# marcinp7/music-style-transfer

Hardware: AMD Instinct MI355X
Metric: style-transfer opt iters/sec (higher is better)
Workload: dtype f32; 1 GPU; one 30 s clip per GPU (BASELINE.json configs[1]): piano-roll C=4,R=16,T=4 (+percussion), full widths (980325 params), fwd+loss+bwd every step, Adam+StepLR every iter_size steps; clips_per_gpu=1, iter_size=2, hip_graph=True, graphs=one joint graph, accumulation=2 concurrent streams, launches_per_pass=71, parallelism=single GPU

## Files before the change

include/mst_amd.h:

```cpp
#ifndef MST_AMD_H
#define MST_AMD_H
#include <stdint.h>

#ifdef __cplusplus
extern "C" {
#endif

typedef enum {
    MST_OK = 0,
    MST_ERR_ARG = -1,
    MST_ERR_UNSUPPORTED = -2,
    MST_ERR_LAUNCH = -3,
    MST_ERR_ALLOC = -4,
} mst_status;

typedef struct {
    int32_t C, R, T;
    int32_t beat, bar, nrf;
    int32_t style, melody, rhythm;
    int32_t instr;
    int32_t n_instruments;
    int32_t has_unpitched;
    int32_t clips;
} mst_dims;
// ... 122 lines not shown
                          const int32_t* rows , int32_t n_clips,
                          const mst_row_fields* fields ,
                          int64_t clip_stride, float* ws, mst_stream stream);

#define MST_EVAL_ACC_WORDS (2 + MST_N_LOSSES + 3 * MST_METRIC_WORDS)
int32_t mst_eval_accumulate(const float* losses   ,
                            const double* metrics ,
                            int32_t n_clips, int32_t channels,
                            const int32_t* live   ,
                            double* acc , mst_stream stream);

int32_t mst_plan_step_count(const mst_plan* p, int32_t stage_mask, int32_t backward);
int32_t mst_plan_step_info(const mst_plan* p, int32_t stage_mask, int32_t backward, int32_t* info );
int32_t mst_plan_step_carried(const mst_plan* p, int32_t stage_mask, int32_t backward, int32_t* carried);
int32_t mst_plan_step_riders(const mst_plan* p, int32_t stage_mask, int32_t backward, int32_t* out);
int32_t mst_plan_zero_rides(const mst_plan* p);
int32_t mst_plan_step_carrier(const mst_plan* p, int32_t stage_mask, int32_t backward, int32_t* out);
int32_t mst_plan_set_lstm_small(mst_plan* p, int32_t on);
int32_t mst_plan_step_gemms(const mst_plan* p, int32_t stage_mask, int32_t backward, int32_t step, int32_t* out, int32_t cap);
int32_t mst_plan_time_steps(const mst_plan* p, int32_t stage_mask, int32_t backward, const float* params,
                            float* gparams, float* ws, const float* pitched, const float* unpitched,
                            mst_stream stream, int32_t reps, float* ms, int32_t* kind, double* flops, double* bytes);

typedef struct mst_audio_plan mst_audio_plan;
mst_audio_plan* mst_audio_plan_create(int32_t n_fft , int32_t hop, int64_t n_samples, int32_t* status);
void mst_audio_plan_destroy(mst_audio_plan* p);
int32_t mst_audio_plan_info(const mst_audio_plan* p, int64_t out[6]);
int32_t mst_audio_stft(const mst_audio_plan* p, const float* audio, float* spec, float* mag, mst_stream stream);
int32_t mst_audio_gram(const mst_audio_plan* p, const float* feat, float* gram, float* ws, mst_stream stream);
int32_t mst_audio_style_iteration(const mst_audio_plan* p, float* x, const float* gram_style, float* grad, float* exp_avg,
                                  float* exp_avg_sq, float* state, float* ws, float* loss, double lr, mst_stream stream);

int32_t mst_debug_slab_columns_disjoint(int64_t off_x, int32_t width_x, int64_t off_y, int32_t width_y, int32_t ld);

const char* mst_version(void);

#ifdef __cplusplus
}
#endif
#endif
```

music-style-transfer_amd/csrc/gemm.hip:

```cpp
#include "combine_body.h"
#include "lstm_small_body.h"

__device__ __forceinline__ float act_fwd(int act, float z, int col) {
    if (act == ACT_LEAKY) return z > 0.f ? z : z * LEAKY;
    if (act == ACT_SIGOUT) { float s = 1.f / (1.f + expf(-z)); return col == 0 ? 6.f * s : s; }
    if (act == ACT_BPM) { float s = 1.f / (1.f + expf(-z)); return s * 150.f + 50.f; }
    return z;
}

__device__ __forceinline__ float act_bwd(int act, float y, int col) {
    if (act == ACT_LEAKY) return y > 0.f ? 1.f : LEAKY;
    if (act == ACT_SIGOUT) return col == 0 ? y * (1.f - y * (1.f / 6.f)) : y * (1.f - y);
    if (act == ACT_BPM) { float s = (y - 50.f) * (1.f / 150.f); return 150.f * s * (1.f - s); }
    return 1.f;
}

typedef const MST_GLOBAL_AS float* gcptr;
#define GEMM_PAD 1

template <int KIND>
__device__ __forceinline__ int off_of(const Operand& o, int i, int j, bool& ok) {
    if constexpr (KIND == OPK_DENSE) {
        return i * (int)o.si + j * (int)o.sj;
    } else if constexpr (KIND == OPK_ACTGRAD) {
        return o.transposed ? j * o.ld + i : i * o.ld + j;
    } else if constexpr (KIND == OPK_IM2COL) {
        const int p = i >> 3, oc = i & 7;
        const int f = j / (CONV_K * NPF), rem = j - f * (CONV_K * NPF);
        const int e = (NDEG * oc - CONV_PAD) * NPF + rem;
        ok = ok & (e >= 0) & (e < NPN * NPF);
        return p * (NF * NPN * NPF) + f * (NPN * NPF) + e;
    } else if constexpr (KIND == OPK_PERMW) {
        if (o.pb == CONV_K && o.pc == NPF) {
            constexpr int BC = CONV_K * NPF;
            const int a = i / BC, rem = i - a * BC;
            const int bb = rem / NPF, c = rem - bb * NPF;
            return j * o.ld + a * BC + c * CONV_K + bb;
        }
        if (o.pb == NUN && o.pc == NUF) {
            constexpr int BC = NUN * NUF;
            const int a = i / BC, rem = i - a * BC;
            const int bb = rem / NUF, c = rem - bb * NUF;
            return j * o.ld + a * BC + c * NUN + bb;
        }
        const int bc = o.pb * o.pc;
        const int a = i / bc, rem = i - a * bc;
        const int bb = rem / o.pc, c = rem - bb * o.pc;
        return j * o.ld + a * bc + c * o.pb + bb;
    } else {
        return (j >> 3) * (o.oc * NOCT) + i * NOCT + (j & 7);
    }
}

template <int OK>
__device__ __forceinline__ void store_out(const GemmDesc& d, float* cbase, const float* bias, int m, int n, int split, float acc) {
    const OutSpec& o = d.out;
    if constexpr (OK == OUT_STORE) {
        float v = acc;
        if (bias) v += o.bias_div > 0 ? bias[(unsigned)((m / o.bias_div) * o.bias_ld + n)] : bias[n];
        cbase[(unsigned)(m * o.ldc + n)] = act_fwd(o.act, v, n);
    } else if constexpr (OK == OUT_ACCUM) {
        float* c = cbase + (unsigned)(m * o.ldc + n);
        *c = o.first ? acc : *c + acc;
    } else if constexpr (OK == OUT_CONV) {
        cbase[(unsigned)((m >> 3) * o.ldc + n * NOCT + (m & 7))] = act_fwd(ACT_LEAKY, acc + bias[n], 0);
    } else if constexpr (OK == OUT_SLAB) {
        const unsigned idx = n < o.wcols ? (unsigned)(m * o.wcols + n) : (unsigned)(d.M * o.wcols + m);
        cbase[(int64_t)split * o.slab_stride + idx] = acc;
    } else {
        unsigned idx;
        if (n < o.wcols) {
            int a, bb, c, bc;
            if (o.pb == CONV_K && o.pc == NPF) { bc = CONV_K * NPF; a = n / (CONV_K * NPF); const int rem = n - a * (CONV_K * NPF); bb = rem / NPF; c = rem - bb * NPF; }
            else if (o.pb == NUN && o.pc == NUF) { bc = NUN * NUF; a = n / (NUN * NUF); const int rem = n - a * (NUN * NUF); bb = rem / NUF; c = rem - bb * NUF; }
            else { bc = o.pb * o.pc; a = n / bc; const int rem = n - a * bc; bb = rem / o.pc; c = rem - bb * o.pc; }
            idx = (unsigned)(m * o.wcols + a * bc + c * o.pb + bb);
        } else {
            idx = (unsigned)(d.M * o.wcols + m);
        }
        cbase[(int64_t)split * o.slab_stride + idx] = acc;
    }
}

template <int AK, int BKIND, int OK, int AKF, int BKF, int KD>
__device__ __forceinline__ void gemm_body(const GemmDesc& d, const Bases& b, const int tile, const int split,
                                          float (*As)[GEMM_BM + GEMM_PAD], float (*Bs)[GEMM_BN + GEMM_PAD]) {
    const int tid = threadIdx.x;
    const int M = d.M, N = d.N;
    const int tiles_n = (N + GEMM_BN - 1) / GEMM_BN;
    const gcptr baseA = (gcptr)(b.p[d.A.space] + d.A.off);
    const gcptr baseA2 = (AK == OPK_ACTGRAD || AK == OPK_CONVGRAD) ? (gcptr)(b.p[d.A.space2] + d.A.off2) : baseA;
    const gcptr baseB = (gcptr)(b.p[d.B.space] + d.B.off);
    const int tm = tile / tiles_n, tn = tile - tm * tiles_n;
    int kchunk = (d.K + d.ksplit - 1) / d.ksplit;
    kchunk = (kchunk + KD - 1) / KD * KD;
    const int k0 = split * kchunk;
    const int k1 = min(d.K, k0 + kchunk);
    const int wv = tid >> 6, lane = tid & 63;
    const int a_act = (AK == OPK_ACTGRAD) ? d.A.act : ACT_LEAKY;
    const int a_tr = d.A.transposed;
    const int b_ones = (BKIND == OPK_DENSE || BKIND == OPK_IM2COL) ? d.B.ones_at : -1;
    typedef float acc_f32x16 __attribute__((ext_vector_type(16)));
    acc_f32x16 acc;
#pragma unroll
    for (int r = 0; r < 16; ++r) acc[r] = 0.f;

    constexpr int NT = GEMM_THREADS, NW = NT / 64;
    constexpr int NL = GEMM_BM * KD / NT;
    constexpr int KW = KD / NW;
    float va[NL], ya[NL], vb[NL];

#define A_ROW(i) (AKF ? (tid / KD) + (NT / KD) * (i) : (tid & 31))
#define A_KL(i) (AKF ? (tid % KD) : (tid >> 5) + (NT / 32) * (i))
#define B_ROW(i) (BKF ? (tid / KD) + (NT / KD) * (i) : (tid & 31))
#define B_KL(i) (BKF ? (tid % KD) : (tid >> 5) + (NT / 32) * (i))
#define GEMM_ISSUE(KT)                                                                                     \
    {                                                                                                      \
        _Pragma("unroll") for (int i = 0; i < NL; ++i) {                                                   \
            const int m = tm * GEMM_BM + A_ROW(i), ka = (KT) + A_KL(i);                                    \
            bool oka = (m < M) & (ka < k1);                                                                \
            int ia = off_of<AK>(d.A, m, ka, oka);                                                          \
            ia = oka ? ia : 0;                                                                             \
            const float x = baseA[(unsigned)ia];                                                           \
            if constexpr (AK == OPK_ACTGRAD || AK == OPK_CONVGRAD) {                                       \
                const float y = baseA2[(unsigned)ia];                                                      \
                const int col = (AK == OPK_ACTGRAD) ? (a_tr ? m : ka) : 0;                                 \
                ya[i] = act_bwd(a_act, y, col);                                                            \
            } else ya[i] = 1.f;                                                                            \
            va[i] = oka ? x : 0.f;                                                                         \
            const int n = tn * GEMM_BN + B_ROW(i), kb = (KT) + B_KL(i);                                    \
            bool okb = (n < N) & (kb < k1);                                                                \
            const bool one = okb & (n == b_ones);                                                          \
            int ib = off_of<BKIND>(d.B, kb, n, okb);                                                       \
            ib = (okb & !one) ? ib : 0;                                                                    \
            const float w = baseB[(unsigned)ib];                                                           \
            vb[i] = one ? 1.f : (okb ? w : 0.f);                                                           \
        }                                                                                                  \
    }

    if (k0 < k1) GEMM_ISSUE(k0)
    for (int kt = k0; kt < k1; kt += KD) {
#pragma unroll
        for (int i = 0; i < NL; ++i) {
            As[A_KL(i)][A_ROW(i)] = (AK == OPK_ACTGRAD || AK == OPK_CONVGRAD) ? va[i] * ya[i] : va[i];
            Bs[B_KL(i)][B_ROW(i)] = vb[i];
        }
        __syncthreads();
        if (kt + KD < k1) GEMM_ISSUE(kt + KD)
#pragma unroll
        for (int kk = 0; kk < KW; kk += 2) {
            const int k = wv * KW + kk + (lane >> 5);
            acc = __builtin_amdgcn_mfma_f32_32x32x2f32(As[k][lane & 31], Bs[k][lane & 31], acc, 0, 0, 0);
        }
        __syncthreads();
    }
#undef GEMM_ISSUE
#undef A_ROW
#undef A_KL
#undef B_ROW
#undef B_KL
    float* red = &As[0][0];
#pragma unroll
    for (int r = 0; r < 16; ++r)
        red[wv * (GEMM_BM * GEMM_BN) + ((r & 3) + 8 * (r >> 2) + 4 * (lane >> 5)) * GEMM_BN + (lane & 31)] = acc[r];
    __syncthreads();
    float* cbase = b.p[d.out.space] + d.out.off;
    const float* bias = d.out.bias_space >= 0 ? b.p[d.out.bias_space] + d.out.bias_off : nullptr;
#pragma unroll
    for (int q = 0; q < GEMM_BM * GEMM_BN / NT; ++q) {
        const int o = tid + q * NT;
// ... 496 lines not shown
        return;
    }
    lb -= seg_blocks;
    if (lb < gat_blocks) {
        const int m = lb / r.gat_blocks;
        gather_rows<GATHER_RIDER_ROWS>(r.gathers[clip * r.gat_members + m], lb - m * r.gat_blocks, r.gat_blocks, b);
        return;
    }
    lb -= gat_blocks;
    if (lb < r.zero_chunks) {
        const ZeroChunk c = r.zero[lb];
        float* p = b.p[SP_GRAD] + (int64_t)clip * r.zero_stride + c.off;
        for (int i = threadIdx.x; i < c.len; i += GEMM_THREADS) p[i] = 0.f;
    }
}

__global__ __launch_bounds__(GEMM_THREADS) void gemm_kernel(const GemmDesc* __restrict__ descs, const int* __restrict__ owner, int count, int blocks_per_clip, int rider_blocks, Bases b, GemmRiders r) {
    constexpr int TILE_F = GEMM_BK * (GEMM_BM + GEMM_PAD), RED_F = (GEMM_THREADS / 64) * GEMM_BM * GEMM_BN;
    __shared__ __attribute__((aligned(16))) float smem[(2 * TILE_F > RED_F) ? 2 * TILE_F : RED_F];
    float (*As)[GEMM_BM + GEMM_PAD] = reinterpret_cast<float (*)[GEMM_BM + GEMM_PAD]>(smem);
    float (*Bs)[GEMM_BN + GEMM_PAD] = reinterpret_cast<float (*)[GEMM_BN + GEMM_PAD]>(smem + TILE_F);
    const int clip = blockIdx.x / blocks_per_clip;
    int lb = blockIdx.x - clip * blocks_per_clip;
    if (lb < rider_blocks) {
        gemm_rider_block(r, clip, lb, b, smem);
        return;
    }
    lb -= rider_blocks;
    const int lo = owner[lb];
    const GemmDesc d = descs[clip * count + lo];
    const int local = lb - d.blk_begin;
    const int ntile = ((d.M + GEMM_BM - 1) / GEMM_BM) * ((d.N + GEMM_BN - 1) / GEMM_BN);
    const int tile = local % ntile, split = local / ntile;
#define GEMM_CASE(V, A_, B_, O_, AF_, BF_)                                                          \
    case (V) * 3 + 0: gemm_body<A_, B_, O_, AF_, BF_, 32>(d, b, tile, split, As, Bs); break;           \
    case (V) * 3 + 1: gemm_body<A_, B_, O_, AF_, BF_, 64>(d, b, tile, split, As, Bs); break;           \
    case (V) * 3 + 2: gemm_body<A_, B_, O_, AF_, BF_, 128>(d, b, tile, split, As, Bs); break;
    switch (d.variant * 3 + d.kdsel) {
        GEMM_CASE(GV_LIN_FWD, OPK_DENSE, OPK_DENSE, OUT_STORE, 1, 1)
        GEMM_CASE(GV_LIN_FWD_PERM, OPK_DENSE, OPK_PERMW, OUT_STORE, 1, 1)
        GEMM_CASE(GV_LIN_DW, OPK_ACTGRAD, OPK_DENSE, OUT_SLAB, 0, 0)
        GEMM_CASE(GV_LIN_DW_PERM, OPK_ACTGRAD, OPK_DENSE, OUT_PERMW_SLAB, 0, 0)
        GEMM_CASE(GV_LIN_DA, OPK_ACTGRAD, OPK_DENSE, OUT_ACCUM, 1, 0)
        GEMM_CASE(GV_CONV_FWD, OPK_IM2COL, OPK_PERMW, OUT_CONV, 1, 1)
        GEMM_CASE(GV_CONV_DW, OPK_CONVGRAD, OPK_IM2COL, OUT_PERMW_SLAB, 1, 0)
        GEMM_CASE(GV_HH_DW, OPK_DENSE, OPK_DENSE, OUT_SLAB, 0, 0)
        GEMM_CASE(GV_LIN_DA_RAW, OPK_DENSE, OPK_DENSE, OUT_ACCUM, 1, 0)
    default: break;
    }
#undef GEMM_CASE
}

int gemm_variant(const GemmDesc& g) {
    const int a = g.A.kind, bk = g.B.kind, o = g.out.kind;
    if (a == OPK_DENSE && bk == OPK_DENSE && o == OUT_STORE) return GV_LIN_FWD;
    if (a == OPK_DENSE && bk == OPK_PERMW && o == OUT_STORE) return GV_LIN_FWD_PERM;
    if (a == OPK_ACTGRAD && bk == OPK_DENSE && o == OUT_SLAB) return GV_LIN_DW;
    if (a == OPK_ACTGRAD && bk == OPK_DENSE && o == OUT_PERMW_SLAB) return GV_LIN_DW_PERM;
    if (a == OPK_ACTGRAD && bk == OPK_DENSE && o == OUT_ACCUM) return GV_LIN_DA;
    if (a == OPK_IM2COL && bk == OPK_PERMW && o == OUT_CONV) return GV_CONV_FWD;
    if (a == OPK_CONVGRAD && bk == OPK_IM2COL && o == OUT_PERMW_SLAB) return GV_CONV_DW;
    if (a == OPK_DENSE && bk == OPK_DENSE && o == OUT_SLAB) return GV_HH_DW;
    if (a == OPK_DENSE && bk == OPK_DENSE && o == OUT_ACCUM) return GV_LIN_DA_RAW;
    return -1;
}

int gemm_rider_blocks(const GemmRiders& r) { return r.lstm_members * r.lstm_blocks + r.comb[0].sites * r.comb[0].blocks + r.comb[1].sites * r.comb[1].blocks + (r.seg_groups + 3) / 4 + r.gat_members * r.gat_blocks + r.zero_chunks; }

int launch_gemm(const GemmDesc* dev_descs, const int* dev_owner, int members, int blocks_per_clip, int clips, int mfma, Bases b, hipStream_t s, const GemmRiders* riders) {
    if (members <= 0 || blocks_per_clip <= 0 || clips <= 0) return 0;
    GemmRiders r = riders ? *riders : GemmRiders{};
    if (mfma && gemm_rider_blocks(r)) return (int)hipErrorInvalidValue;
    blocks_per_clip += gemm_rider_blocks(r);
    if (mfma) hipLaunchKernelGGL(gemm_mfma_kernel, dim3(blocks_per_clip * clips), dim3(MF_THREADS), 0, s, dev_descs, dev_owner, members, blocks_per_clip, b);
    else hipLaunchKernelGGL(gemm_kernel, dim3(blocks_per_clip * clips), dim3(GEMM_THREADS), 0, s, dev_descs, dev_owner, members, blocks_per_clip, gemm_rider_blocks(r), b, r);
    return (int)hipGetLastError();
}

template <int WV>
__device__ __forceinline__ void gather_rows(const GatherDesc& d, const int blk, const int nblk, const Bases& b) {
    const int lane = threadIdx.x & 63, wv = (threadIdx.x >> 6) & (WV - 1);
    for (int row = blk * WV + wv; row < d.rows; row += nblk * WV) {
        unsigned t = (unsigned)row;
        int rc[4];
        rc[3] = t % (unsigned)d.d[3]; t /= (unsigned)d.d[3];
        rc[2] = t % (unsigned)d.d[2]; t /= (unsigned)d.d[2];
        rc[1] = t % (unsigned)d.d[1]; rc[0] = t / (unsigned)d.d[1];
        float* out = b.p[SP_WS] + d.out_off + (int64_t)row * d.K;
        if (d.sum) {
            for (int w = lane; w < d.K; w += 64) {
                float a = 0.f;
                for (int sIdx = 0; sIdx < d.nseg; ++sIdx) {
                    const Seg& sg = d.seg[sIdx];
// ... 219 lines not shown
```

music-style-transfer_amd/csrc/mst_common.h:

```cpp
#pragma once
#include <hip/hip_runtime.h>
#include <stdint.h>

#include "../../include/mst_amd.h"

#ifndef MST_GLOBAL_AS
#define MST_GLOBAL_AS __attribute__((address_space(1)))
#endif
#ifndef MST_CONST_AS
#define MST_CONST_AS __attribute__((address_space(4)))
#endif
#ifndef MST_UNIFORM
#define MST_UNIFORM(x) __builtin_amdgcn_readfirstlane(x)
#endif
#ifndef MST_FAST_EXP
#define MST_FAST_EXP(x) __expf(x)
#define MST_FAST_RCP(x) __builtin_amdgcn_rcpf(x)
#define MST_PIN(x) asm volatile("" : "+v"(x))
#endif
#ifndef MST_PIN_SGPR
#if defined(__AMDGCN__)
#define MST_PIN_SGPR(p) asm volatile("" : "+s"(p))
#else
#define MST_PIN_SGPR(p) ((void)(p))
// ... 219 lines not shown
int launch_lin_dx(const LinDesc& d, Bases b, int first, hipStream_t s);
int launch_lin_dw(const LinDesc& d, Bases b, hipStream_t s);
int lin_dw_tiles(const LinDesc& d);

struct RowLinDesc {
    int32_t rows, kin, nout, act, xgrad;
    int64_t x_off, y_off;
    int64_t w_off, b_off;
    int64_t slab_off; int32_t slab_stride, nblk;
    int32_t first;
};

struct CopyDesc { int64_t src_off, dst_off; int32_t na, nb, cols, src_sa, src_sb, dst_sa, dst_sb, first; };
struct FoldDesc { int32_t space, nrows, row_stride, ncols, col_stride, pad; int64_t part_off, sum_off ; };
int launch_copy_rows(const CopyDesc* dev, const CopyDesc& host, int backward, Bases b, hipStream_t s);
int launch_fold(const FoldDesc* dev, int spread, Bases b, hipStream_t s);
int launch_combine_phase(const CombineDesc* dev, int nblk, int which, Bases b, hipStream_t s, int count = 1, int mc4 = 0, int whole_small = 0);

struct SlabEntry { int64_t dst, src, stride; int32_t count, splits; int32_t reps; int64_t rep_stride; int32_t width, dst_ld; int32_t single;
                   int64_t base;  };
struct SlabBlock { int32_t entry, start; };

struct Sizes {
    int OC, PCE_IL, H, HB;
    int SE_L, SE_IL, SE_ML, SE_BL;
    int ME_BL, ME_BRL, ME_IL, ME_CW, MEL;
    int RH, PRE_BL, PRE_BRL, PRE_CL, PRE_IL, PRE_ML, PRE_BPL, URE_CL;
    int SIM_BL, NRF, SIM_SI, SIM_RI, SIM_SM, SIM_RM, SIM_SB, SIM_RB, NI;
    int PSA_SL, PSA_RL, PSA_IL, PSA_ML, USA_SL, USA_RL;
    int I, STYLE, BAR;
};
Sizes mst_sizes(const mst_dims& d);

enum { GV_LIN_FWD, GV_LIN_FWD_PERM, GV_LIN_DW, GV_LIN_DW_PERM, GV_LIN_DA, GV_CONV_FWD, GV_CONV_DW, GV_HH_DW, GV_LIN_DA_RAW };
int launch_gather(const GatherDesc* dev, int count, int max_rows, Bases b, hipStream_t s);
int gemm_variant(const GemmDesc& g);
int launch_gemm(const GemmDesc* dev_descs, const int* dev_owner, int members, int blocks_per_clip, int clips, int mfma, Bases b, hipStream_t s,
                const GemmRiders* riders = nullptr);
int gemm_rider_blocks(const GemmRiders& r);
int gemm_tile_edge(int mfma);
int gemm_blocks(const GemmDesc& g, int mfma);
int launch_segred(const SegRedDesc* dev_descs, int members, int blocks_per_clip, int clips, int stage2_blocks, Bases b, hipStream_t s);
int launch_segred2(const SegRedDesc* dev_descs, int count, int stage2_blocks, Bases b, hipStream_t s);
int launch_lstm_transpose(const LstmDesc* dev_descs, int count, int maxH, int multi, Bases b, hipStream_t s);
int launch_lstm_fwd(const LstmDesc* dev_descs, int count, int maxB, int maxH, int multi, int small, Bases b, hipStream_t s);
int launch_lstm_bwd(const LstmDesc* dev_descs, int count, int maxB, int maxH, int multi, int small, Bases b, hipStream_t s);
bool lstm_small(int count, int maxB, int maxH);
int lstm_multi_blocks_per_cu();
int launch_combine_fwd(const CombineDesc* dev_descs, int count, int max_nblk, int all_small, int mc4, Bases b, hipStream_t s);
int launch_combine_bwd(const CombineDesc* dev_descs, int count, int max_nblk, int all_small, int mc4, Bases b, hipStream_t s);
int launch_me_sumsq(const NotesDesc* dev, const NotesDesc& host, int count, Bases b, hipStream_t s);
int launch_me_notes_fwd(const NotesDesc* dev, const NotesDesc& host, int count, Bases b, hipStream_t s);
int launch_me_bwd_reduce(const NotesDesc* dev, const NotesDesc& host, int count, Bases b, hipStream_t s);
int launch_me_notes_bwd(const NotesDesc* dev, const NotesDesc& host, int count, Bases b, hipStream_t s);
int launch_psa_notes_fwd(const NotesDesc* dev, const NotesDesc& host, int count, Bases b, hipStream_t s);
int launch_psa_notes_bwd(const NotesDesc* dev, const NotesDesc& host, int count, Bases b, hipStream_t s);
int psa_bwd_waves(int C);
struct LossBatch { int32_t clips; int64_t ws, grad, tmp, ext0, ext1; };
int loss_fwd_partials(const float* pp, const float* pt, int64_t np, const float* up, const float* ut, int64_t nu, float* scratch,
                      hipStream_t s);
int loss_fwd_tail(int64_t np, int64_t nu, int has_u, const float* il, const float* it, int ni, const float* mlg, const float* mt,
                  const float* bp, const float* bt, int normalize, float* losses, float* saved, float* scratch, hipStream_t s,
                  float* gl_onehot, float* losses_out);
int loss_blocks(int64_t n);
int loss_fwd_batched(const float* pp, const float* pt, int64_t np, const float* up, const float* ut, int64_t nu, const float* il,
                     const float* it, int ni, const float* mlg, const float* mt, const float* bp, const float* bt, int normalize,
                     float* losses, float* saved, float* scratch, LossBatch lb, hipStream_t s,
// ... 31 lines not shown
```

music-style-transfer_amd/csrc/plan.hip:

```cpp
#include <cmath>
#include <cstdio>
#include <cstdlib>
#include <cstring>
#include <map>
#include <string>
#include <array>
#include <vector>

#include "mst_common.h"

#define MST_ALIGN_UP(n) (((n) + 63) / 64 * 64)

static int mean_size(double a, double b, double factor = 1.0) { return (int)std::ceil(((a + b) / 2.0) * factor); }

Sizes mst_sizes(const mst_dims& d) {
    Sizes z{};
    z.I = d.instr; z.STYLE = d.style; z.BAR = d.bar; z.H = d.beat; z.HB = d.bar / 2; z.RH = d.rhythm;
    z.MEL = d.melody; z.NRF = d.nrf; z.NI = d.n_instruments;
    z.OC = mean_size(NF * NPF, d.beat);
    z.PCE_IL = mean_size(d.instr, d.beat);
    z.SE_L = mean_size(d.bar, d.style);
    z.SE_IL = mean_size(d.instr, d.style, .25);
    z.SE_ML = mean_size(2, d.style, .1);
    z.SE_BL = mean_size(d.style, 1, .05);
    z.ME_BL = mean_size(d.beat, d.melody);
    z.ME_BRL = mean_size(d.bar, d.melody);
    z.ME_IL = mean_size(d.instr, d.melody, .25);
    z.ME_CW = mean_size(NPF, d.melody);
    z.PRE_BL = mean_size(d.beat, d.rhythm);
    z.PRE_BRL = mean_size(d.bar, d.rhythm, .5);
    z.PRE_CL = mean_size(NPN * NPF, d.rhythm, .1);
    z.PRE_IL = mean_size(d.instr, d.rhythm, .5);
// ... 1251 lines not shown
    const int n = (int)seq.size();
    std::vector<std::vector<Acc>> acc(n);
    std::vector<int> level(n, 0);
    int maxlevel = 0;
    for (int i = 0; i < n; ++i) {
        accesses(seq[i], acc[i]);
        for (int j = 0; j < i; ++j)
            if (level[j] >= level[i] && conflicts(acc[i], acc[j])) level[i] = level[j] + 1;
        if (level[i] > maxlevel) maxlevel = level[i];
    }
    std::vector<char> done(n, 0);
    for (int lv = 0; lv <= maxlevel; ++lv) {
        const size_t lv_begin = out.size();
        for (int i = 0; i < n; ++i) {
            if (done[i] || level[i] != lv) continue;
            const Step& s0 = seq[i];
            const KindInfo& ki = KINDS[s0.kind];
            const bool mergeable = !opt.no_merge && ki.merge, is_lstm = ki.fam == F_LSTM;
            Step m = s0; m.count = 0; m.lvl = lv;
            std::vector<int> members;
            for (int j = i; j < n; ++j) {
                if (done[j] || level[j] != lv) continue;
                const Step& s = seq[j];
                if (s.kind != s0.kind || (!across_stages && s.stage != s0.stage)) continue;
                if (is_lstm && lstm_band(s.b) != lstm_band(s0.b)) continue;
                if (is_lstm && j != i && (lstms.host[s.first].multi || lstms.host[s0.first].multi)) continue;
                if (j != i && !mergeable) continue;
                done[j] = 1;
                for (int q = 0; q < s.count; ++q) members.push_back(s.first + q);
                m.stage |= s.stage;
                if (s.a > m.a) m.a = s.a;
                if (s.b > m.b) m.b = s.b;
            }
            const bool shared_T = s0.kind == K_LSTM_T && !lstms.host[s0.first].multi;
            const int reps = ki.per_clip && !shared_T ? K() : 1;
            if (ki.sched)
                with_sched_table(ki.fam, [&](auto& t) {
                    m.first = (int)t.sched.size();
                    for (int k = 0; k < reps; ++k)
                        for (int idx : members) t.sched.push_back(reloc(t.host[idx], k));
                });
            m.count = (int)members.size() * reps;
            if (ki.fam == F_GEMM) {
                for (int q = 0; q < m.count; ++q) {
                    GemmDesc& g = gemms.sched[m.first + q];
                    g.variant = gemm_variant(g);
                    if (g.fold_rows) {
                        g.acs = shift(g.A.space, 1); g.acs2 = (g.A.kind == OPK_ACTGRAD || g.A.kind == OPK_CONVGRAD) ? shift(g.A.space2, 1) : 0; g.bcs = shift(g.B.space, 1);
                        if ((uint64_t)std::max(g.acs, std::max(g.acs2, g.bcs)) * (uint64_t)K() > 0xFFFFFFFFull) err = MST_ERR_UNSUPPORTED;
                    }
                    if (g.clip_rows) {
                        g.M = K();
                        if (g.A.kind == OPK_DENSE) g.A.si = shift(g.A.space, 1);
                        else g.A.ld = (int32_t)shift(g.A.space, 1);
                        g.out.ldc = (int32_t)shift(g.out.space, 1);
                        if ((uint64_t)act_top * (uint64_t)K() > 0x7FFFFFFFull) err = MST_ERR_UNSUPPORTED;
                    }
                    const int kr = (g.K + g.ksplit - 1) / g.ksplit;
                    g.kdsel = kr <= 32 ? 0 : (kr <= 64 ? 1 : 2);
                    g.run = (mfma && opt.gemm_run > 1) ? opt.gemm_run : 1;
                    if (g.variant < 0) err = MST_ERR_UNSUPPORTED;
                }
                const int nm = (int)members.size();
                int total = 0;
                m.c = (int)s_gemm_owner.size();
                for (int q = 0; q < nm; ++q) {
// ... 794 lines not shown
}

extern "C" int32_t mst_plan_step_info(const mst_plan* p, int32_t mask, int32_t backward, int32_t* info ) {
    if (!p || !info) return MST_ERR_ARG;
    int idx = 0;
    for (const Step* s : steps_of(p, mask, backward)) {
        int32_t* o = info + 8 * idx++;
        o[0] = o[1] = o[2] = o[3] = 0; o[4] = s->count; o[5] = s->kind; o[6] = s->lvl; o[7] = s->chain;
        if (s->kind == K_GEMM || s->kind == K_GEMM_FOLD) { const GemmDesc& g = p->gemms.sched[s->first]; o[0] = g.M; o[1] = g.N; o[2] = g.K; o[3] = g.ksplit; }
        else if (KINDS[s->kind].fam == F_LIN) { const LinDesc& l = p->lins.host[s->first]; o[0] = l.rows; o[1] = l.N; o[2] = l.K; o[3] = l.splits; }
        else if (s->kind == K_LSTM_F || s->kind == K_LSTM_B) { const LstmDesc& l = p->lstms.sched[s->first]; o[0] = l.B; o[1] = l.S; o[2] = l.H; o[3] = l.multi; }
        else if (s->kind == K_GATHER) { const GatherDesc& g = p->gathers.sched[s->first]; o[0] = g.rows; o[1] = g.K; o[2] = g.nseg; }
        else if (s->kind == K_SEGRED) { const SegRedDesc& r = p->segreds.sched[s->first]; o[0] = s->a; o[1] = r.width; o[2] = r.d[0] * r.d[1] * r.d[2] * r.d[3]; }
        else if (s->kind == K_COMB_F || s->kind == K_COMB_B) { const CombineDesc& c = p->combines.sched[s->first]; o[0] = c.Cn; o[1] = c.rows; o[2] = c.cols; o[3] = c.nblk; }
    }
    return idx;
}

extern "C" int32_t mst_plan_step_gemms(const mst_plan* p, int32_t mask, int32_t backward, int32_t step, int32_t* out, int32_t cap) {
    if (!p || !out) return MST_ERR_ARG;
    const std::vector<const Step*> steps = steps_of(p, mask, backward);
    if (step < 0 || step >= (int)steps.size()) return MST_ERR_ARG;
    const Step& s = *steps[step];
    if (s.kind != K_GEMM && s.kind != K_GEMM_FOLD) return 0;
    int n = 0;
    for (int q = 0; q < s.b && n < cap; ++q, ++n) {
        const GemmDesc& g = p->gemms.sched[s.first + q];
        int32_t* o = out + 6 * n;
        o[0] = g.M; o[1] = g.N; o[2] = g.K; o[3] = g.ksplit; o[4] = g.fold_rows; o[5] = gemm_blocks(g, p->mfma);
    }
    return n;
}

extern "C" int32_t mst_plan_time_steps(const mst_plan* p, int32_t mask, int32_t backward, const float* params, float* gparams,
                                       float* ws, const float* pitched, const float* unpitched, mst_stream stream,
                                       int32_t reps, float* ms, int32_t* kind, double* flops, double* bytes) {
    if (!p || !params || !ws || !ms || !kind || !flops || !bytes || reps < 1) return MST_ERR_ARG;
    hipStream_t st = (hipStream_t)stream;
    Bases b = make_bases(p, params, gparams, ws, pitched, unpitched);
    if (backward && !p->tiled()) b.flags = MST_BF_LOSS_FUSED;
    if ((mask & MST_STAGE_ALL) == MST_STAGE_ALL) b.flags |= MST_BF_ALL_STAGES;
    hipEvent_t e0, e1;
    if (hipEventCreate(&e0) != hipSuccess || hipEventCreate(&e1) != hipSuccess) return MST_ERR_ALLOC;
    const std::vector<Step>& L = p->list(mask, backward);
    int idx = 0;
    for (const Step* s : steps_of(p, mask, backward)) {
        float t = 0.f;
        if (s->carrier < 0) {
            run_step(p, L, *s, b, st);
            hipEventRecord(e0, st);
            for (int r = 0; r < reps; ++r) run_step(p, L, *s, b, st);
            hipEventRecord(e1, st);
            hipEventSynchronize(e1);
            hipEventElapsedTime(&t, e0, e1);
        }
        ms[idx] = t / reps; kind[idx] = s->kind == K_GEMM_FOLD ? K_GEMM : s->kind;
        step_cost(p, *s, &flops[idx], &bytes[idx]);
        ++idx;
    }
    hipEventDestroy(e0); hipEventDestroy(e1);
    return idx;
}

extern "C" const char* mst_version(void) { return "mst_amd 0.1 (gfx950)"; }
```

music-style-transfer_amd/style/_native.py:

```python
import collections
import ctypes as C
import os

import torch

_HERE = os.path.dirname(os.path.abspath(__file__))
DEFAULT_LIB = os.path.join(os.path.dirname(_HERE), 'libmst_amd.so')

STAGE_EXTRACT, STAGE_INFO, STAGE_APPLY, STAGE_ALL = 1, 2, 4, 7
LOSS_SAVED = 512
LOSS_KEYS = [
    'total', 'channels_loss_total', 'channels_loss_pitched_total', 'channels_loss_pitched_notes_loss',
    'channels_loss_pitched_velocity_loss', 'channels_loss_pitched_duration_loss',
    'channels_loss_pitched_accidentals_loss', 'channels_loss_unpitched_total',
    'channels_loss_unpitched_notes_loss', 'channels_loss_unpitched_velocity_loss',
    'channels_loss_unpitched_duration_loss', 'song_info_loss_total', 'song_info_loss_instruments_loss',
    'song_info_loss_mode_loss', 'song_info_loss_bpm_loss',
]
N_LOSSES = len(LOSS_KEYS)


class MstError(RuntimeError):
    pass

# ... 82 lines not shown
    'mst_train_iteration': (C.c_int32, [_P, _P, _P, _P, _P, _P, _P, _P]),
    'mst_tiled_phase_count': (C.c_int32, [_P]),
    'mst_tiled_phase': (C.c_int32, [_P, C.c_int32, _P, _P, _P, _P, _P, _P, C.c_int32, _P, C.POINTER(C.c_int64 * 8), C.POINTER(C.c_int64 * 8),
                        C.POINTER(C.c_int32)]),
    'mst_adam_step': (C.c_int32, [_P, _P, _P, _P, C.c_int64, _P, C.c_double, C.c_double, C.c_double, C.c_double,
                                  C.c_int32, C.c_double, C.c_int32, _P]),
    'mst_adam_step2': (C.c_int32, [_P, _P, _P, _P, _P, C.c_int64, _P, C.c_double, C.c_double, C.c_double, C.c_double,
                                   C.c_int32, C.c_double, C.c_int32, _P]),
    'mst_grad_guard_scratch_bytes': (C.c_int64, [C.c_int64]),
    'mst_grad_norm': (C.c_int32, [_P, _P, C.c_int64, _P, _P, _P]),
    'mst_grad_norms': (C.c_int32, [_P, _P, _P, _P, C.c_int32, _P, _P]),
    'mst_adam_step_guarded': (C.c_int32, [_P, _P, _P, _P, _P, C.c_int64, _P, _P, _P, C.c_double, C.c_double, C.c_double, C.c_double,
                                          C.c_int32, C.c_double, C.c_double, C.c_int32, C.c_int32, _P]),
    'mst_hard_output': (C.c_int32, [_P, _P, C.c_int64, C.c_int32, _P]),
    'mst_clip_scatter': (C.c_int32, [_P, _P, _P, C.c_int32, C.c_int32, C.c_int64, C.c_int32, _P, _P]),
    'mst_clip_window': (C.c_int32, [_P, _P, _P, C.c_int32, C.c_int32, C.c_int32, C.c_int64, C.c_int32, _P, _P]),
    'mst_roll_slices': (C.c_int64, [C.c_int64]),
    'mst_roll_count': (C.c_int32, [_P, C.c_int64, C.c_int32, C.c_int32, _P, _P]),
    'mst_roll_compact': (C.c_int32, [_P, C.c_int64, C.c_int32, C.c_int32, _P, C.c_int64, _P, _P, _P]),
    'mst_roll_metrics_scratch_bytes': (C.c_int64, [C.c_int64, C.c_int64]),
    'mst_roll_metrics': (C.c_int32, [_P, _P, C.c_int64, C.c_int64, C.c_int32, _P, _P, _P]),
    'mst_eval_scratch_bytes': (C.c_int64, [_P]),
    'mst_eval_iteration': (C.c_int32, [_P, _P, _P, _P, _P, _P, _P, _P, _P]),
    'mst_window_inputs': (C.c_int32, [_P, C.c_int32, C.c_int32, _P, C.c_int32, C.POINTER(RowFields), C.c_int64, _P, _P]),
    'mst_eval_accumulate': (C.c_int32, [_P, _P, C.c_int32, C.c_int32, _P, _P, _P]),
    'mst_plan_step_count': (C.c_int32, [_P, C.c_int32, C.c_int32]),
    'mst_plan_step_info': (C.c_int32, [_P, C.c_int32, C.c_int32, _P]),
    'mst_plan_step_carried': (C.c_int32, [_P, C.c_int32, C.c_int32, _P]),
    'mst_plan_step_riders': (C.c_int32, [_P, C.c_int32, C.c_int32, _P]),
    'mst_plan_zero_rides': (C.c_int32, [_P]),
    'mst_plan_step_carrier': (C.c_int32, [_P, C.c_int32, C.c_int32, _P]),
    'mst_plan_set_lstm_small': (C.c_int32, [_P, C.c_int32]),
    'mst_plan_step_gemms': (C.c_int32, [_P, C.c_int32, C.c_int32, C.c_int32, _P, C.c_int32]),
    'mst_plan_time_steps': (C.c_int32, [_P, C.c_int32, C.c_int32, _P, _P, _P, _P, _P, _P, C.c_int32, _P, _P, _P, _P]),
    'mst_audio_plan_create': (_P, [C.c_int32, C.c_int32, C.c_int64, C.POINTER(C.c_int32)]),
    'mst_audio_plan_destroy': (None, [_P]),
    'mst_audio_plan_info': (C.c_int32, [_P, C.POINTER(C.c_int64 * 6)]),
    'mst_audio_stft': (C.c_int32, [_P, _P, _P, _P, _P]),
    'mst_audio_gram': (C.c_int32, [_P, _P, _P, _P, _P]),
    'mst_audio_style_iteration': (C.c_int32, [_P, _P, _P, _P, _P, _P, _P, _P, _P, C.c_double, _P]),
    'mst_version': (C.c_char_p, []),
}


def ptr(t):
    if t is None:
        return None
    if t.dtype != torch.float32 or not t.is_contiguous():
        raise MstError('mst_amd kernels take contiguous float32 tensors')
    return t.data_ptr()


def check(status, what):
    if status != 0:
        names = {-1: 'MST_ERR_ARG', -2: 'MST_ERR_UNSUPPORTED', -3: 'MST_ERR_LAUNCH', -4: 'MST_ERR_ALLOC'}
        raise MstError(f'{what} failed: {names.get(status, status)}')


class Native:
    def __init__(self, path=None):
        path = path or DEFAULT_LIB
        if not os.path.exists(path):
            raise MstError(
                f'{path} not found: the HIP library has not been built. Run `python -c "import __graft_entry__ as g; '
                f'g.build()"` (hipcc --offload-arch=gfx950). There is no CPU fallback.')
        self.path = path
# ... 214 lines not shown
        got = self.lib.mst_plan_step_carried(self.handle, mask, int(backward), out.ctypes.data)
        check(got if got < 0 else 0, 'mst_plan_step_carried')
        return out.tolist()

    def step_riders(self, mask=STAGE_ALL, backward=False):
        import numpy as np
        n = self.lib.mst_plan_step_count(self.handle, mask, int(backward))
        out = np.zeros(n, np.int32)
        got = self.lib.mst_plan_step_riders(self.handle, mask, int(backward), out.ctypes.data)
        check(got if got < 0 else 0, 'mst_plan_step_riders')
        return out.tolist()

    def step_carrier(self, mask=STAGE_ALL, backward=False):
        import numpy as np
        n = self.lib.mst_plan_step_count(self.handle, mask, int(backward))
        out = np.zeros(n, np.int32)
        got = self.lib.mst_plan_step_carrier(self.handle, mask, int(backward), out.ctypes.data)
        check(got if got < 0 else 0, 'mst_plan_step_carrier')
        return out.tolist()

    def set_lstm_small(self, on):
        check(self.lib.mst_plan_set_lstm_small(self.handle, int(on)), 'mst_plan_set_lstm_small')

    def zero_rides(self):
        got = self.lib.mst_plan_zero_rides(self.handle)
        check(got if got < 0 else 0, 'mst_plan_zero_rides')
        return got

    def step_gemms(self, mask, backward, step, cap=2048):
        import numpy as np
        out = np.zeros((cap, 6), np.int32)
        n = self.lib.mst_plan_step_gemms(self.handle, mask, int(backward), step, out.ctypes.data, cap)
        check(n if n < 0 else 0, 'mst_plan_step_gemms')
        return [tuple(r) for r in out[:n].tolist()]

    def tiled_train_iteration(self, params, gparams, pitched, unpitched, losses=None, is_root=True, all_reduce=None):
        if all_reduce is None:
            import torch.distributed as dist
            all_reduce = lambda t: dist.all_reduce(t, op=dist.ReduceOp.SUM)
        xoff, xlen, nx = (C.c_int64 * 8)(), (C.c_int64 * 8)(), C.c_int32()
        self._touch(None)
        for ph in range(self.lib.mst_tiled_phase_count(self.handle)):
            check(self.lib.mst_tiled_phase(self.handle, ph, ptr(params), ptr(gparams), ptr(self.ws), ptr(pitched), ptr(unpitched),
                                           ptr(losses), int(bool(is_root)), current_stream(self.device), C.byref(xoff), C.byref(xlen),
                                           C.byref(nx)), f'mst_tiled_phase({ph})')
            if nx.value == 1:
                all_reduce(self.ws[xoff[0]:xoff[0] + xlen[0]])
            elif nx.value > 1:
                parts = [self.ws[xoff[q]:xoff[q] + xlen[q]] for q in range(nx.value)]
                total = sum(int(xlen[q]) for q in range(nx.value))
                if getattr(self, '_xstage', None) is None or self._xstage.numel() < total:
                    self._xstage = torch.empty(total, dtype=torch.float32, device=self.device)
                stage = self._xstage[:total]
                torch.cat(parts, out=stage)
                all_reduce(stage)
                at = 0
                for t in parts:
                    t.copy_(stage[at:at + t.numel()])
                    at += t.numel()

    def train_iteration(self, params, gparams, pitched, unpitched, losses=None, ws=None):
        check(self.lib.mst_train_iteration(self.handle, ptr(params), ptr(gparams), ptr(self._touch(ws)),
                                           ptr(pitched), ptr(unpitched), ptr(losses), current_stream(self.device)),
              'mst_train_iteration')

    def eval_scratch(self):
# ... 25 lines not shown
```

Baseline: 2839 iters/s.

## Walk GEMM operand offsets incrementally and sort merged GEMM members by cost

```diff
diff --git a/include/mst_amd.h b/include/mst_amd.h
--- a/include/mst_amd.h
+++ b/include/mst_amd.h
@@ -178,6 +178,9 @@
                                   float* exp_avg_sq, float* state, float* ws, float* loss, double lr, mst_stream stream);
 
 int32_t mst_debug_slab_columns_disjoint(int64_t off_x, int32_t width_x, int64_t off_y, int32_t width_y, int32_t ld);
+int64_t mst_debug_gemm_walk(int32_t kind, int32_t as_b, int32_t rows, int32_t K, int32_t k0, int32_t k1, int32_t kd, int32_t ld,
+                            int32_t pb, int32_t pc, int32_t oc, int64_t* compared);
+int32_t mst_plan_step_gemm_kinds(const mst_plan* p, int32_t stage_mask, int32_t backward, int32_t step, int32_t* out, int32_t cap);
 
 const char* mst_version(void);
 
diff --git a/music-style-transfer_amd/csrc/gemm.hip b/music-style-transfer_amd/csrc/gemm.hip
--- a/music-style-transfer_amd/csrc/gemm.hip
+++ b/music-style-transfer_amd/csrc/gemm.hip
@@ -19,7 +19,7 @@
 #define GEMM_PAD 1
 
 template <int KIND>
-__device__ __forceinline__ int off_of(const Operand& o, int i, int j, bool& ok) {
+__host__ __device__ __forceinline__ int off_of(const Operand& o, int i, int j, bool& ok) {
     if constexpr (KIND == OPK_DENSE) {
         return i * (int)o.si + j * (int)o.sj;
     } else if constexpr (KIND == OPK_ACTGRAD) {
@@ -50,6 +50,153 @@
     } else {
         return (j >> 3) * (o.oc * NOCT) + i * NOCT + (j & 7);
     }
+}
+
+template <int KF, int KD> __host__ __device__ __forceinline__ int walk_row(int tid, int i) { return KF ? tid / KD + (GEMM_THREADS / KD) * i : (tid & 31); }
+template <int KF, int KD> __host__ __device__ __forceinline__ int walk_kl(int tid, int i) { return KF ? tid % KD : (tid >> 5) + (GEMM_THREADS / 32) * i; }
+template <int PERM> struct PermOf { static constexpr int PB = PERM == 1 ? CONV_K : NUN, PC = PERM == 1 ? NPF : NUF; };
+__host__ __device__ __forceinline__ int perm_case(int pb, int pc) { return (pb == CONV_K && pc == NPF) ? 1 : ((pb == NUN && pc == NUF) ? 2 : 0); }
+
+template <int KIND, bool ISB, int KF, int KD, int PERM>
+struct OpWalk {
+    int tid, r0, R;
+    __host__ __device__ __forceinline__ void init(const Operand&, int tid_, int r0_, int R_, int) { tid = tid_; r0 = r0_; R = R_; }
+    __host__ __device__ __forceinline__ void advance() {}
+    __host__ __device__ __forceinline__ int at(const Operand& o, int i, int kt, int k1, bool& inb, bool& ok) const {
+        const int r = r0 + walk_row<KF, KD>(tid, i), k = kt + walk_kl<KF, KD>(tid, i);
+        inb = (r < R) & (k < k1);
+        ok = inb;
+        return ISB ? off_of<KIND>(o, k, r, ok) : off_of<KIND>(o, r, k, ok);
+    }
+};
+template <int KD, int PERM>
+struct OpWalk<OPK_IM2COL, false, 1, KD, PERM> {
+    static constexpr int BC = CONV_K * NPF, ROWS = GEMM_THREADS / KD;
+    static_assert(ROWS % NOCT == 0, "a lane's rows share their octave");
+    int m0, R, kl, rem, e0, off0;
+    __host__ __device__ __forceinline__ void init(const Operand&, int tid, int r0, int R_, int k0) {
+        m0 = r0 + tid / KD; R = R_; kl = tid % KD;
+        const int j = k0 + kl, f = j / BC;
+        rem = j - f * BC;
+        e0 = (NDEG * (m0 & 7) - CONV_PAD) * NPF;
+        off0 = (m0 >> 3) * (NF * NPN * NPF) + f * (NPN * NPF) + e0 + rem;
+    }
+    __host__ __device__ __forceinline__ void advance() {
+        rem += KD % BC; off0 += (KD / BC) * (NPN * NPF) + KD % BC;
+        if (rem >= BC) { rem -= BC; off0 += NPN * NPF - BC; }
+    }
+    __host__ __device__ __forceinline__ int at(const Operand&, int i, int kt, int k1, bool& inb, bool& ok) const {
+        const int e = e0 + rem;
+        inb = (m0 + ROWS * i < R) & (kt + kl < k1);
+        ok = inb & (e >= 0) & (e < NPN * NPF);
+        return off0 + i * (ROWS / NOCT) * (NF * NPN * NPF);
+    }
+};
+template <int KD, int PERM>
+struct OpWalk<OPK_IM2COL, true, 0, KD, PERM> {
+    static constexpr int BC = CONV_K * NPF;
+    static_assert(KD % NOCT == 0, "a k-tile is whole positions");
+    int kl, off0; bool colok, padok;
+    __host__ __device__ __forceinline__ void init(const Operand&, int tid, int r0, int R, int k0) {
+        const int n = r0 + (tid & 31), f = n / BC, rem = n - f * BC;
+        kl = tid >> 5;
+        const int k = k0 + kl, e = (NDEG * (k & 7) - CONV_PAD) * NPF + rem;
+        colok = n < R;
+        padok = (e >= 0) & (e < NPN * NPF);
+        off0 = (k >> 3) * (NF * NPN * NPF) + f * (NPN * NPF) + e;
+    }
+    __host__ __device__ __forceinline__ void advance() { off0 += (KD / NOCT) * (NF * NPN * NPF); }
+    __host__ __device__ __forceinline__ int at(const Operand&, int i, int kt, int k1, bool& inb, bool& ok) const {
+        inb = colok & (kt + kl + (GEMM_THREADS / 32) * i < k1);
+        ok = inb & padok;
+        return off0 + i * (GEMM_THREADS / 32 / NOCT) * (NF * NPN * NPF);
+    }
+};
+template <int KD, int PERM>
+struct OpWalk<OPK_PERMW, true, 1, KD, PERM> {
+    static constexpr int PB = PermOf<PERM>::PB, PC = PermOf<PERM>::PC, BC = PB * PC, ROWS = GEMM_THREADS / KD;
+    static constexpr int DA = KD / BC, DB = KD % BC / PC, DC = KD % BC % PC;
+    static_assert(PERM == 1 || PERM == 2, "one of the model's two permutations");
+    int n0, R, kl, c, bb, off0, rstep;
+    __host__ __device__ __forceinline__ void init(const Operand& o, int tid, int r0, int R_, int k0) {
+        n0 = r0 + tid / KD; R = R_; kl = tid % KD;
+        const int j = k0 + kl, a = j / BC, rem = j - a * BC;
+        bb = rem / PC; c = rem - bb * PC;
+        off0 = n0 * o.ld + a * BC + c * PB + bb;
+        rstep = ROWS * o.ld;
+    }
+    __host__ __device__ __forceinline__ void advance() {
+        c += DC; bb += DB; off0 += DA * BC + DC * PB + DB;
+        if (c >= PC) { c -= PC; bb += 1; off0 += 1 - BC; }
+        if (bb >= PB) { bb -= PB; off0 += BC - PB; }
+    }
+    __host__ __device__ __forceinline__ int at(const Operand&, int i, int kt, int k1, bool& inb, bool& ok) const {
+        inb = (n0 + ROWS * i < R) & (kt + kl < k1);
+        ok = inb;
+        return off0 + i * rstep;
+    }
+};
+template <int KD, int PERM>
+struct OpWalk<OPK_CONVGRAD, false, 1, KD, PERM> {
+    static constexpr int ROWS = GEMM_THREADS / KD;
+    static_assert(KD % NOCT == 0, "a k-tile is whole positions");
+    int m0, R, kl, off0, kstep;
+    __host__ __device__ __forceinline__ void init(const Operand& o, int tid, int r0, int R_, int k0) {
+        m0 = r0 + tid / KD; R = R_; kl = tid % KD;
+        const int j = k0 + kl;
+        off0 = (j >> 3) * (o.oc * NOCT) + m0 * NOCT + (j & 7);
+        kstep = (KD / NOCT) * (o.oc * NOCT);
+    }
+    __host__ __device__ __forceinline__ void advance() { off0 += kstep; }
+    __host__ __device__ __forceinline__ int at(const Operand&, int i, int kt, int k1, bool& inb, bool& ok) const {
+        inb = (m0 + ROWS * i < R) & (kt + kl < k1);
+        ok = inb;
+        return off0 + i * ROWS * NOCT;
+    }
+};
+
+template <int KIND, bool ISB, int KF, int KD, int PERM>
+static int64_t walk_mismatches(const Operand& o, int rows, int k0, int k1, int64_t* compared) {
+    constexpr int NL = GEMM_BM * KD / GEMM_THREADS;
+    int64_t bad = 0, seen = 0;
+    for (int r0 = 0; r0 < rows; r0 += GEMM_BM)
+        for (int tid = 0; tid < GEMM_THREADS; ++tid) {
+            OpWalk<KIND, ISB, KF, KD, PERM> w;
+            w.init(o, tid, r0, rows, k0);
+            for (int kt = k0; kt < k1; kt += KD) {
+                for (int i = 0; i < NL; ++i) {
+                    bool inb, ok;
+                    const int off = w.at(o, i, kt, k1, inb, ok);
+                    const int r = r0 + walk_row<KF, KD>(tid, i), k = kt + walk_kl<KF, KD>(tid, i);
+                    const bool rinb = (r < rows) & (k < k1);
+                    bool rok = rinb;
+                    const int roff = ISB ? off_of<KIND>(o, k, r, rok) : off_of<KIND>(o, r, k, rok);
+                    bad += (inb != rinb) | (ok != rok) | (rinb & (off != roff));
+                    ++seen;
+                }
+                w.advance();
+            }
+        }
+    if (compared) *compared = seen;
+    return bad;
+}
+
+extern "C" int64_t mst_debug_gemm_walk(int32_t kind, int32_t as_b, int32_t rows, int32_t K, int32_t k0, int32_t k1, int32_t kd,
+                                       int32_t ld, int32_t pb, int32_t pc, int32_t oc, int64_t* compared) {
+    if (rows < 1 || K < 1 || k0 < 0 || k0 % 8 || k1 > K || k0 > k1 || (kd != 32 && kd != 64 && kd != 128)) return MST_ERR_ARG;
+    Operand o{};
+    o.kind = kind; o.ld = ld; o.pb = pb; o.pc = pc; o.oc = oc; o.ones_at = -1;
+#define WALK_KD(KIND, ISB, KF, PERM)                                                                      \
+    return kd == 32 ? walk_mismatches<KIND, ISB, KF, 32, PERM>(o, rows, k0, k1, compared)                 \
+                    : (kd == 64 ? walk_mismatches<KIND, ISB, KF, 64, PERM>(o, rows, k0, k1, compared)     \
+                                : walk_mismatches<KIND, ISB, KF, 128, PERM>(o, rows, k0, k1, compared));
+    if (kind == OPK_IM2COL && !as_b) { WALK_KD(OPK_IM2COL, false, 1, 0) }
+    if (kind == OPK_IM2COL && as_b) { WALK_KD(OPK_IM2COL, true, 0, 0) }
+    if (kind == OPK_CONVGRAD && !as_b) { WALK_KD(OPK_CONVGRAD, false, 1, 0) }
+    if (kind == OPK_PERMW && as_b && perm_case(pb, pc) == 1) { WALK_KD(OPK_PERMW, true, 1, 1) }
+    if (kind == OPK_PERMW && as_b && perm_case(pb, pc) == 2) { WALK_KD(OPK_PERMW, true, 1, 2) }
+#undef WALK_KD
+    return MST_ERR_UNSUPPORTED;
 }
 
 template <int OK>
@@ -82,7 +229,7 @@
     }
 }
 
-template <int AK, int BKIND, int OK, int AKF, int BKF, int KD>
+template <int AK, int BKIND, int OK, int AKF, int BKF, int KD, int PERM = 0>
 __device__ __forceinline__ void gemm_body(const GemmDesc& d, const Bases& b, const int tile, const int split,
                                           float (*As)[GEMM_BM + GEMM_PAD], float (*Bs)[GEMM_BN + GEMM_PAD]) {
     const int tid = threadIdx.x;
@@ -110,32 +257,38 @@
     constexpr int KW = KD / NW;
     float va[NL], ya[NL], vb[NL];
 
-#define A_ROW(i) (AKF ? (tid / KD) + (NT / KD) * (i) : (tid & 31))
-#define A_KL(i) (AKF ? (tid % KD) : (tid >> 5) + (NT / 32) * (i))
-#define B_ROW(i) (BKF ? (tid / KD) + (NT / KD) * (i) : (tid & 31))
-#define B_KL(i) (BKF ? (tid % KD) : (tid >> 5) + (NT / 32) * (i))
+#define A_ROW(i) walk_row<AKF, KD>(tid, i)
+#define A_KL(i) walk_kl<AKF, KD>(tid, i)
+#define B_ROW(i) walk_row<BKF, KD>(tid, i)
+#define B_KL(i) walk_kl<BKF, KD>(tid, i)
+    OpWalk<AK, false, AKF, KD, PERM> wa;
+    OpWalk<BKIND, true, BKF, KD, PERM> wb;
+    wa.init(d.A, tid, tm * GEMM_BM, M, k0);
+    wb.init(d.B, tid, tn * GEMM_BN, N, k0);
 #define GEMM_ISSUE(KT)                                                                                     \
     {                                                                                                      \
         _Pragma("unroll") for (int i = 0; i < NL; ++i) {                                                   \
-            const int m = tm * GEMM_BM + A_ROW(i), ka = (KT) + A_KL(i);                                    \
-            bool oka = (m < M) & (ka < k1);                                                                \
-            int ia = off_of<AK>(d.A, m, ka, oka);                                                          \
+            bool ina, oka;                                                                                 \
+            int ia = wa.at(d.A, i, (KT), k1, ina, oka);                                                    \
             ia = oka ? ia : 0;                                                                             \
             const float x = baseA[(unsigned)ia];                                                           \
             if constexpr (AK == OPK_ACTGRAD || AK == OPK_CONVGRAD) {                                       \
                 const float y = baseA2[(unsigned)ia];                                                      \
-                const int col = (AK == OPK_ACTGRAD) ? (a_tr ? m : ka) : 0;                                 \
+                int col = 0;                                                                               \
+                if constexpr (AK == OPK_ACTGRAD) col = a_tr ? tm * GEMM_BM + A_ROW(i) : (KT) + A_KL(i);    \
                 ya[i] = act_bwd(a_act, y, col);                                                            \
             } else ya[i] = 1.f;                                                                            \
             va[i] = oka ? x : 0.f;                                                                         \
-            const int n = tn * GEMM_BN + B_ROW(i), kb = (KT) + B_KL(i);                                    \
-            bool okb = (n < N) & (kb < k1);                                                                \
-            const bool one = okb & (n == b_ones);                                                          \
-            int ib = off_of<BKIND>(d.B, kb, n, okb);                                                       \
+            bool inb, okb;                                                                                 \
+            int ib = wb.at(d.B, i, (KT), k1, inb, okb);                                                    \
+            bool one = false;                                                                              \
+            if constexpr (BKIND == OPK_DENSE || BKIND == OPK_IM2COL) one = inb & (tn * GEMM_BN + B_ROW(i) == b_ones); \
             ib = (okb & !one) ? ib : 0;                                                                    \
             const float w = baseB[(unsigned)ib];                                                           \
             vb[i] = one ? 1.f : (okb ? w : 0.f);                                                           \
         }                                                                                                  \
+        wa.advance();                                                                                      \
+        wb.advance();                                                                                      \
     }
 
     if (k0 < k1) GEMM_ISSUE(k0)
@@ -698,33 +851,39 @@
     const int local = lb - d.blk_begin;
     const int ntile = ((d.M + GEMM_BM - 1) / GEMM_BM) * ((d.N + GEMM_BN - 1) / GEMM_BN);
     const int tile = local % ntile, split = local / ntile;
-#define GEMM_CASE(V, A_, B_, O_, AF_, BF_)                                                          \
-    case (V) * 3 + 0: gemm_body<A_, B_, O_, AF_, BF_, 32>(d, b, tile, split, As, Bs); break;           \
-    case (V) * 3 + 1: gemm_body<A_, B_, O_, AF_, BF_, 64>(d, b, tile, split, As, Bs); break;           \
-    case (V) * 3 + 2: gemm_body<A_, B_, O_, AF_, BF_, 128>(d, b, tile, split, As, Bs); break;
-    switch (d.variant * 3 + d.kdsel) {
+#define GEMM_CASE_P(V, A_, B_, O_, AF_, BF_, P_)                                                    \
+    case (V) * 3 + 0: gemm_body<A_, B_, O_, AF_, BF_, 32, P_>(d, b, tile, split, As, Bs); break;       \
+    case (V) * 3 + 1: gemm_body<A_, B_, O_, AF_, BF_, 64, P_>(d, b, tile, split, As, Bs); break;       \
+    case (V) * 3 + 2: gemm_body<A_, B_, O_, AF_, BF_, 128, P_>(d, b, tile, split, As, Bs); break;
+#define GEMM_CASE(V, A_, B_, O_, AF_, BF_) GEMM_CASE_P(V, A_, B_, O_, AF_, BF_, 0)
+    int sel = d.variant * 3 + d.kdsel;
+    if (d.variant == GV_LIN_FWD_PERM && perm_case(d.B.pb, d.B.pc) == 2) sel = GV_COUNT * 3 + d.kdsel;
+    switch (sel) {
         GEMM_CASE(GV_LIN_FWD, OPK_DENSE, OPK_DENSE, OUT_STORE, 1, 1)
-        GEMM_CASE(GV_LIN_FWD_PERM, OPK_DENSE, OPK_PERMW, OUT_STORE, 1, 1)
+        GEMM_CASE_P(GV_LIN_FWD_PERM, OPK_DENSE, OPK_PERMW, OUT_STORE, 1, 1, 1)
+        GEMM_CASE_P(GV_COUNT, OPK_DENSE, OPK_PERMW, OUT_STORE, 1, 1, 2)
         GEMM_CASE(GV_LIN_DW, OPK_ACTGRAD, OPK_DENSE, OUT_SLAB, 0, 0)
         GEMM_CASE(GV_LIN_DW_PERM, OPK_ACTGRAD, OPK_DENSE, OUT_PERMW_SLAB, 0, 0)
         GEMM_CASE(GV_LIN_DA, OPK_ACTGRAD, OPK_DENSE, OUT_ACCUM, 1, 0)
-        GEMM_CASE(GV_CONV_FWD, OPK_IM2COL, OPK_PERMW, OUT_CONV, 1, 1)
+        GEMM_CASE_P(GV_CONV_FWD, OPK_IM2COL, OPK_PERMW, OUT_CONV, 1, 1, 1)
         GEMM_CASE(GV_CONV_DW, OPK_CONVGRAD, OPK_IM2COL, OUT_PERMW_SLAB, 1, 0)
         GEMM_CASE(GV_HH_DW, OPK_DENSE, OPK_DENSE, OUT_SLAB, 0, 0)
         GEMM_CASE(GV_LIN_DA_RAW, OPK_DENSE, OPK_DENSE, OUT_ACCUM, 1, 0)
     default: break;
     }
+#undef GEMM_CASE_P
 #undef GEMM_CASE
 }
 
 int gemm_variant(const GemmDesc& g) {
     const int a = g.A.kind, bk = g.B.kind, o = g.out.kind;
     if (a == OPK_DENSE && bk == OPK_DENSE && o == OUT_STORE) return GV_LIN_FWD;
+    if (bk == OPK_PERMW && !perm_case(g.B.pb, g.B.pc)) return -1;
     if (a == OPK_DENSE && bk == OPK_PERMW && o == OUT_STORE) return GV_LIN_FWD_PERM;
     if (a == OPK_ACTGRAD && bk == OPK_DENSE && o == OUT_SLAB) return GV_LIN_DW;
     if (a == OPK_ACTGRAD && bk == OPK_DENSE && o == OUT_PERMW_SLAB) return GV_LIN_DW_PERM;
     if (a == OPK_ACTGRAD && bk == OPK_DENSE && o == OUT_ACCUM) return GV_LIN_DA;
-    if (a == OPK_IM2COL && bk == OPK_PERMW && o == OUT_CONV) return GV_CONV_FWD;
+    if (a == OPK_IM2COL && bk == OPK_PERMW && o == OUT_CONV) return perm_case(g.B.pb, g.B.pc) == 1 ? GV_CONV_FWD : -1;
     if (a == OPK_CONVGRAD && bk == OPK_IM2COL && o == OUT_PERMW_SLAB) return GV_CONV_DW;
     if (a == OPK_DENSE && bk == OPK_DENSE && o == OUT_SLAB) return GV_HH_DW;
     if (a == OPK_DENSE && bk == OPK_DENSE && o == OUT_ACCUM) return GV_LIN_DA_RAW;
diff --git a/music-style-transfer_amd/csrc/mst_common.h b/music-style-transfer_amd/csrc/mst_common.h
--- a/music-style-transfer_amd/csrc/mst_common.h
+++ b/music-style-transfer_amd/csrc/mst_common.h
@@ -275,7 +275,7 @@
 };
 Sizes mst_sizes(const mst_dims& d);
 
-enum { GV_LIN_FWD, GV_LIN_FWD_PERM, GV_LIN_DW, GV_LIN_DW_PERM, GV_LIN_DA, GV_CONV_FWD, GV_CONV_DW, GV_HH_DW, GV_LIN_DA_RAW };
+enum { GV_LIN_FWD, GV_LIN_FWD_PERM, GV_LIN_DW, GV_LIN_DW_PERM, GV_LIN_DA, GV_CONV_FWD, GV_CONV_DW, GV_HH_DW, GV_LIN_DA_RAW, GV_COUNT };
 int launch_gather(const GatherDesc* dev, int count, int max_rows, Bases b, hipStream_t s);
 int gemm_variant(const GemmDesc& g);
 int launch_gemm(const GemmDesc* dev_descs, const int* dev_owner, int members, int blocks_per_clip, int clips, int mfma, Bases b, hipStream_t s,
diff --git a/music-style-transfer_amd/csrc/plan.hip b/music-style-transfer_amd/csrc/plan.hip
--- a/music-style-transfer_amd/csrc/plan.hip
+++ b/music-style-transfer_amd/csrc/plan.hip
@@ -1,3 +1,4 @@
+#include <algorithm>
 #include <cmath>
 #include <cstdio>
 #include <cstdlib>
@@ -1315,6 +1316,25 @@
                 if (s.a > m.a) m.a = s.a;
                 if (s.b > m.b) m.b = s.b;
             }
+            if (ki.fam == F_GEMM && !mfma && !opt.no_merge) {
+                auto ktiles = [&](int idx) {
+                    const GemmDesc& g = gemms.host[idx];
+                    const int kr = (g.K + g.ksplit - 1) / g.ksplit, kd = kr <= 32 ? 32 : (kr <= 64 ? 64 : 128);
+                    return (kr + kd - 1) / kd;
+                };
+                auto dear = [&](int idx) {
+                    switch (gemm_variant(gemms.host[idx])) {
+                    case GV_CONV_FWD: case GV_CONV_DW: return 3;
+                    case GV_LIN_FWD_PERM: case GV_LIN_DW_PERM: return 2;
+                    case GV_LIN_DW: case GV_LIN_DA: return 1;
+                    default: return 0;
+                    }
+                };
+                std::stable_sort(members.begin(), members.end(), [&](int x, int y) {
+                    const int kx = ktiles(x), ky = ktiles(y);
+                    return kx != ky ? kx > ky : dear(x) > dear(y);
+                });
+            }
             const bool shared_T = s0.kind == K_LSTM_T && !lstms.host[s0.first].multi;
             const int reps = ki.per_clip && !shared_T ? K() : 1;
             if (ki.sched)
@@ -2175,6 +2195,20 @@
     return n;
 }
 
+extern "C" int32_t mst_plan_step_gemm_kinds(const mst_plan* p, int32_t mask, int32_t backward, int32_t step, int32_t* out, int32_t cap) {
+    if (!p || !out) return MST_ERR_ARG;
+    const std::vector<const Step*> steps = steps_of(p, mask, backward);
+    if (step < 0 || step >= (int)steps.size()) return MST_ERR_ARG;
+    const Step& s = *steps[step];
+    if (s.kind != K_GEMM && s.kind != K_GEMM_FOLD) return 0;
+    int n = 0;
+    for (int q = 0; q < s.b && n < cap; ++q, ++n) {
+        const GemmDesc& g = p->gemms.sched[s.first + q];
+        out[2 * n] = g.variant; out[2 * n + 1] = p->mfma ? 32 : 32 << g.kdsel;
+    }
+    return n;
+}
+
 extern "C" int32_t mst_plan_time_steps(const mst_plan* p, int32_t mask, int32_t backward, const float* params, float* gparams,
                                        float* ws, const float* pitched, const float* unpitched, mst_stream stream,
                                        int32_t reps, float* ms, int32_t* kind, double* flops, double* bytes) {
diff --git a/music-style-transfer_amd/style/_native.py b/music-style-transfer_amd/style/_native.py
--- a/music-style-transfer_amd/style/_native.py
+++ b/music-style-transfer_amd/style/_native.py
@@ -138,6 +138,8 @@
     'mst_plan_step_carrier': (C.c_int32, [_P, C.c_int32, C.c_int32, _P]),
     'mst_plan_set_lstm_small': (C.c_int32, [_P, C.c_int32]),
     'mst_plan_step_gemms': (C.c_int32, [_P, C.c_int32, C.c_int32, C.c_int32, _P, C.c_int32]),
+    'mst_plan_step_gemm_kinds': (C.c_int32, [_P, C.c_int32, C.c_int32, C.c_int32, _P, C.c_int32]),
+    'mst_debug_gemm_walk': (C.c_int64, [C.c_int32] * 11 + [C.POINTER(C.c_int64)]),
     'mst_plan_time_steps': (C.c_int32, [_P, C.c_int32, C.c_int32, _P, _P, _P, _P, _P, _P, C.c_int32, _P, _P, _P, _P]),
     'mst_audio_plan_create': (_P, [C.c_int32, C.c_int32, C.c_int64, C.POINTER(C.c_int32)]),
     'mst_audio_plan_destroy': (None, [_P]),
@@ -418,6 +420,13 @@
         out = np.zeros((cap, 6), np.int32)
         n = self.lib.mst_plan_step_gemms(self.handle, mask, int(backward), step, out.ctypes.data, cap)
         check(n if n < 0 else 0, 'mst_plan_step_gemms')
+        return [tuple(r) for r in out[:n].tolist()]
+
+    def step_gemm_kinds(self, mask, backward, step, cap=2048):
+        import numpy as np
+        out = np.zeros((cap, 2), np.int32)
+        n = self.lib.mst_plan_step_gemm_kinds(self.handle, mask, int(backward), step, out.ctypes.data, cap)
+        check(n if n < 0 else 0, 'mst_plan_step_gemm_kinds')
         return [tuple(r) for r in out[:n].tolist()]
 
     def tiled_train_iteration(self, params, gparams, pitched, unpitched, losses=None, is_root=True, all_reduce=None):
```

Result: faster. 2889 iters/s (median of 6 runs) (+1.8%).
